# IGLICT/NeRFFaceEditing

Hardware: NVIDIA B200
Metric: rendered rays/sec (48+48 samples) (higher is better)
Workload: dtype f32 (gather, compositing) + bf16x3 split tensor-core MLP with f32 accumulate

## Files before the change

include/nfe_b200.h:

```cpp
#ifndef NFE_B200_H
#define NFE_B200_H

#include <stdint.h>

#ifdef __cplusplus
extern "C" {
#endif

typedef void* nfe_stream_t;

int nfe_version(void);
const char* nfe_last_error(void);
uint64_t nfe_launch_count(void);
int nfe_timing_enable(int on);
int nfe_timing_read(double* ms_by_stage, int64_t* count_by_stage, int n_stages, int reset);

int nfe_bench_l2_gather(const float* table, int64_t n_lines, int warps_per_cta, int depth, int iters, int64_t* host_lines_out,
                        float* sink, nfe_stream_t stream);

int nfe_plane_stats(const float* planes, int64_t n_slabs, int64_t hw, float* mean, float* std_out,
                    nfe_stream_t stream);
int nfe_plane_normalize(const float* planes, const float* mean, const float* std_in, int64_t n_slabs,
                        int64_t hw, float* out, nfe_stream_t stream);
int nfe_plane_denormalize(const float* norm, const float* mean, const float* std_in, int64_t n_slabs,
                          int64_t stat_slabs, int64_t hw, float* out, nfe_stream_t stream);
int nfe_plane_normalize_bwd(const float* g_norm, const float* norm, const float* std_in, const float* g_mean,
                            const float* g_std, int64_t n_slabs, int64_t hw, double* sums_ws, float* g_planes,
                            nfe_stream_t stream);
int nfe_resize_bilinear(const float* in, int64_t n_img, int in_h, int in_w, int out_h, int out_w, int antialias,
                        float* out, nfe_stream_t stream);
int nfe_planes_to_channel_last(const float* planes, int64_t n_img, int channels, int64_t hw, float* out,
                               nfe_stream_t stream);

int nfe_plane_normalize_staged(const float* planes, const float* mean, const float* std_in, int64_t n_img,
                               int64_t hw, float* out_norm, float* out_norm_cl, float* out_raw_cl,
                               nfe_stream_t stream);

int nfe_generate_rays(const float* cam2world , const float* intrinsics , int n,
                      int resolution, float* origins , float* dirs, nfe_stream_t stream);
int nfe_ray_limits_box(const float* origins, const float* dirs, int64_t n_rays, float box_side_length,
                       float* tmin, float* tmax, nfe_stream_t stream);

int nfe_sample_stratified(int64_t n_rays, int s_c, int mode, const float* table, double ray_start,
                          double ray_end, const float* start_per_ray, const float* end_per_ray,
                          const float* jitter, int stochastic, uint64_t seed, uint64_t offset,
                          float* depths , nfe_stream_t stream);

int nfe_sample_planes_fwd(const float* planes_cl, int plane_batch, int channels, int height, int width,
                          const float* coords , int n, int64_t m, float box_warp, float* out,
                          nfe_stream_t stream);

// ... 144 lines not shown
```

nerffaceediting_b200/_lib.py:

```python
import ctypes
import os

_HERE = os.path.dirname(os.path.abspath(__file__))
LIB_PATH = os.path.join(_HERE, "lib", "libnfe_b200.so")

DEC_OSG, DEC_DISENTANGLED, DEC_SEGMENTATION = 0, 1, 2
PREC_FP32, PREC_BF16X3, PREC_BF16 = 0, 1, 2

c_f32p = ctypes.c_void_p
c_i64 = ctypes.c_int64
c_u64 = ctypes.c_uint64
c_int = ctypes.c_int
c_float = ctypes.c_float
c_double = ctypes.c_double
c_vp = ctypes.c_void_p


class NfeMlp(ctypes.Structure):
    _fields_ = [("w1", c_vp), ("b1", c_vp), ("w2", c_vp), ("b2", c_vp),
                ("in_dim", c_int), ("hidden", c_int), ("out_dim", c_int),
                ("wgain1", c_float), ("bgain1", c_float), ("wgain2", c_float), ("bgain2", c_float)]


class NfeRenderCfg(ctypes.Structure):
# ... 13 lines not shown

_MLP_P = ctypes.POINTER(NfeMlp)
_CFG_P = ctypes.POINTER(NfeRenderCfg)

SIGNATURES = {
    "nfe_version": (c_int, []),
    "nfe_last_error": (ctypes.c_char_p, []),
    "nfe_launch_count": (c_u64, []),
    "nfe_timing_enable": (c_int, [c_int]),
    "nfe_timing_read": (c_int, [ctypes.POINTER(c_double), ctypes.POINTER(c_i64), c_int, c_int]),
    "nfe_bench_l2_gather": (c_int, [c_vp, c_i64, c_int, c_int, c_int, ctypes.POINTER(c_i64), c_vp, c_vp]),
    "nfe_plane_stats": (c_int, [c_vp, c_i64, c_i64, c_vp, c_vp, c_vp]),
    "nfe_plane_normalize": (c_int, [c_vp, c_vp, c_vp, c_i64, c_i64, c_vp, c_vp]),
    "nfe_plane_denormalize": (c_int, [c_vp, c_vp, c_vp, c_i64, c_i64, c_i64, c_vp, c_vp]),
    "nfe_plane_normalize_staged": (c_int, [c_vp, c_vp, c_vp, c_i64, c_i64, c_vp, c_vp, c_vp, c_vp]),
    "nfe_planes_to_channel_last": (c_int, [c_vp, c_i64, c_int, c_i64, c_vp, c_vp]),
    "nfe_generate_rays": (c_int, [c_vp, c_vp, c_int, c_int, c_vp, c_vp, c_vp]),
    "nfe_ray_limits_box": (c_int, [c_vp, c_vp, c_i64, c_float, c_vp, c_vp, c_vp]),
    "nfe_sample_stratified": (c_int, [c_i64, c_int, c_int, c_vp, c_double, c_double, c_vp, c_vp, c_vp, c_int, c_u64, c_u64, c_vp, c_vp]),
    "nfe_sample_planes_fwd": (c_int, [c_vp, c_int, c_int, c_int, c_int, c_vp, c_int, c_i64, c_float, c_vp, c_vp]),
    "nfe_decoder_fwd": (c_int, [c_int, c_int, _MLP_P, _MLP_P, c_vp, c_vp, c_int, c_i64, c_int, c_vp, c_vp, c_vp, c_vp]),
    "nfe_composite_fwd": (c_int, [c_vp, c_vp, c_vp, c_vp, c_i64, c_int, c_int, c_int, c_int, c_vp, c_vp, c_vp, c_vp, c_vp, c_vp, c_vp]),
    "nfe_importance_resample": (c_int, [c_vp, c_vp, c_i64, c_int, c_int, c_vp, c_int, c_u64, c_u64, c_vp, c_vp, c_vp, c_vp]),
    "nfe_sample_pdf": (c_int, [c_vp, c_vp, c_i64, c_int, c_int, c_int, c_vp, c_int, c_u64, c_u64, c_float, c_vp, c_vp]),
    "nfe_unify_samples":(c_int, [c_vp] * 8 + [c_i64, c_int, c_int, c_int, c_int] + [c_vp] * 4 + [c_vp]),
    "nfe_render_workspace_bytes": (c_i64, [_CFG_P, c_int, c_i64]),
    "nfe_render_fwd": (c_int, [_CFG_P, _MLP_P, _MLP_P, c_vp, c_vp, c_int, c_vp, c_vp, c_int, c_i64, c_vp, c_vp,
                               c_vp, c_vp, c_vp, c_vp, c_vp, c_int, c_vp, c_vp, c_vp, c_i64, c_vp]),
    "nfe_render_workspace_layout": (c_int, [_CFG_P, c_int, c_i64, ctypes.POINTER(c_i64)]),
    "nfe_composite_bwd": (c_int, [c_vp, c_vp, c_vp, c_int, c_vp, c_vp, c_vp, c_int, c_i64, c_int, c_int, c_vp, c_vp, c_vp, c_vp, c_vp, c_vp, c_vp, c_vp]),
# ... 66 lines not shown
```

nerffaceediting_b200/autograd.py:

```python
import ctypes
import os

import torch
import torch.nn.functional as F

from . import _lib, ops

MAX_ROWS = 1 << 22


def _mlp(x, seq):
    a, b = seq[0], seq[2]
    h = F.softplus(torch.addmm((a.bias * a.bias_gain).unsqueeze(0), x, (a.weight * a.weight_gain).t()))
    return torch.addmm((b.bias * b.bias_gain).unsqueeze(0), h, (b.weight * b.weight_gain).t())


def _decode(kind, seq_a, seq_b, fn, fd):
    if kind == ops.DEC_DISENTANGLED:
        g = _mlp(fn, seq_a)
        return g[:, :1], g[:, 1:], torch.sigmoid(_mlp(fd, seq_b)) * (1 + 2 * 0.001) - 0.001
    x = _mlp(fd, seq_a)
    rgb = torch.sigmoid(x[:, 1:]) * (1 + 2 * 0.001) - 0.001
    return x[:, :1], (_mlp(fd, seq_b) if kind == ops.DEC_SEGMENTATION else None), rgb

# ... 210 lines not shown
        if g.get("rgb") is not None:
            g_rec[:, 16:48] = g["rgb"].reshape(n * m, 32)
        with torch.cuda.device(dev):
            fb = _FieldBackward(kind, seq_a, seq_b, norm_cl, denorm_cl, ctx.affine, ctx.box_warp, ctx.needs_input_grad[5:], dev)
            fb.run_pass(n, rec, g_rec, coords=coords)
            norm_shape, plane_shape = ctx.plane_shapes
            g_norm, g_planes, g_scale, g_shift, g_params = fb.finish(norm_shape, plane_shape, ctx.needs_input_grad[1], ctx.needs_input_grad[2],
                                                                     ctx.stat_shapes, ctx.needs_input_grad[3], ctx.needs_input_grad[4])
        return (None, g_norm, g_planes, g_scale, g_shift) + tuple(g_params)


class NormalizeFunction(torch.autograd.Function):

    @staticmethod
    def forward(ctx, planes):
        mean, std = ops.plane_stats(planes)
        norm_cl = None
        if planes.dim() == 4 and planes.shape[1] == 96 and planes.is_contiguous() and planes.dtype == torch.float32:
            norm, norm_cl, _ = ops.plane_normalize_staged(planes.detach(), mean, std, register=False)
        else:
            norm = ops.plane_normalize(planes, mean, std)
        ctx.save_for_backward(norm, std)
        ctx.hw = planes.shape[-1] * planes.shape[-2]
        if norm_cl is None:
            return norm, mean, std, None
        ctx.mark_non_differentiable(norm_cl)
        return norm, mean, std, norm_cl

    @staticmethod
    def backward(ctx, g_norm, g_mean, g_std, _g_cl=None):
        norm, std = ctx.saved_tensors
        def f32(t):
            return None if t is None else t.contiguous().float()
        g, gm, gs = f32(g_norm), f32(g_mean), f32(g_std)
        slabs = norm.numel() // ctx.hw
        gx = torch.empty_like(norm)
        sums = torch.empty((slabs, 2), device=norm.device, dtype=torch.float64) if g is not None else None
        with torch.cuda.device(norm.device):
            _lib.check(_lib.load().nfe_plane_normalize_bwd(ops._ptr(g), ops._ptr(norm), ops._ptr(std), ops._ptr(gm), ops._ptr(gs), slabs, ctx.hw,
                                                           ops._ptr(sums), ops._ptr(gx), torch.cuda.current_stream(norm.device).cuda_stream),
                       "nfe_plane_normalize_bwd")
        return gx


class DenormalizeFunction(torch.autograd.Function):
# ... 20 lines not shown
```

nerffaceediting_b200/csrc/nfe_march.cu:

```cuda
#include "nfe_march.cuh"

namespace nfe {

__device__ __forceinline__ double shfl_up_double(double v, int delta)
{
    int lo = __double2loint(v), hi = __double2hiint(v);
    lo = __shfl_up_sync(0xffffffffu, lo, delta);
    hi = __shfl_up_sync(0xffffffffu, hi, delta);
    return __hiloint2double(hi, lo);
}
__device__ __forceinline__ double shfl_xor_double(double v, int mask)
{
    int lo = __double2loint(v), hi = __double2hiint(v);
    lo = __shfl_xor_sync(0xffffffffu, lo, mask);
    hi = __shfl_xor_sync(0xffffffffu, hi, mask);
    return __hiloint2double(hi, lo);
}

__device__ __forceinline__ void ray_interval_weights(const float* s_depth, const float* s_sigma, float* s_w, int S, int lane, float& wd, float& wt)
{
    const int n_int = S - 1;
    const int chunk = (n_int + 31) / 32;
    const int i0 = lane * chunk, i1 = min(n_int, i0 + chunk);
    float prod = 1.0f;
    for (int i = i0; i < i1; ++i) {
        const float delta = __fsub_rn(s_depth[i + 1], s_depth[i]);
        const float sig = __fdiv_rn(__fadd_rn(s_sigma[i], s_sigma[i + 1]), 2.0f);
        const float xs = __fsub_rn(sig, 1.0f);
        const float dens = fmaxf(xs, 0.0f) + __logf(1.0f + __expf(-fabsf(xs)));
        const float alpha = __fsub_rn(1.0f, __expf(-__fmul_rn(dens, delta)));
        s_w[i] = alpha;
        prod *= __fadd_rn(__fsub_rn(1.0f, alpha), 1e-10f);
    }
    float incl = prod;
#pragma unroll
    for (int o = 1; o < 32; o <<= 1) {
        const float up = __shfl_up_sync(0xffffffffu, incl, o);
        if (lane >= o) incl *= up;
    }
    float T = __shfl_up_sync(0xffffffffu, incl, 1);
    if (lane == 0) T = 1.0f;
    for (int i = i0; i < i1; ++i) {
        const float alpha = s_w[i];
        const float w = __fmul_rn(alpha, T);
        T *= __fadd_rn(__fsub_rn(1.0f, alpha), 1e-10f);
        s_w[i] = w;
        wd = fmaf(w, __fdiv_rn(__fadd_rn(s_depth[i], s_depth[i + 1]), 2.0f), wd);
        wt = __fadd_rn(wt, w);
    }
}

__device__ __forceinline__ void cp_async16(uint32_t dst_smem, const void* src)
{
    asm volatile("cp.async.cg.shared.global [%0], [%1], 16;" ::"r"(dst_smem), "l"(src) : "memory");
}
__device__ __forceinline__ void cp_async_commit() { asm volatile("cp.async.commit_group;" ::: "memory"); }
template <int N>
__device__ __forceinline__ void cp_async_wait() { asm volatile("cp.async.wait_group %0;" ::"n"(N) : "memory"); }

constexpr int MARCH_RING_GROUPS = 4;
constexpr int MARCH_MIN_BLOCKS = 4;
template <bool SORT>
__global__ void __launch_bounds__(256, MARCH_MIN_BLOCKS) march_kernel(MarchArgs a)
// ... 252 lines not shown
            const bool first = e < a.s1;
            const int64_t row = first ? ray * a.s1 + e : ray * a.s2 + (e - a.s1);
            for (int c = lane; c < a.cc; c += 32) colors_out[(ray * S + k) * a.cc + c] = (first ? a.colors1 : a.colors2)[row * a.cc + c];
            for (int c = lane; c < a.cs; c += 32) segs_out[(ray * S + k) * a.cs + c] = (first ? a.segs1 : a.segs2)[row * a.cs + c];
        }
        __syncwarp();
    }
}

constexpr int RESAMPLE_MIN_BLOCKS = 4;
template <bool SMOOTH>
__global__ void __launch_bounds__(256, RESAMPLE_MIN_BLOCKS) resample_kernel(ResampleArgs a)
{
    extern __shared__ __align__(16) float smem[];
    const int warp = threadIdx.x >> 5, lane = threadIdx.x & 31;
    const int warps_per_block = blockDim.x >> 5;
    const int S = a.S, nw = S - 1, ns = SMOOTH ? S - 3 : a.ns;
    const int per_warp = 4 * S + (a.sort_u ? a.s_f : 0);
    float* s_z = smem + (size_t)warp * per_warp;
    float* s_om = s_z + S;
    float* s_bins = s_om + S;
    float* s_cdf = s_bins + S;
    float* s_u = s_cdf + S;
    for (int64_t ray = (int64_t)blockIdx.x * warps_per_block + warp; ray < a.n_rays; ray += (int64_t)gridDim.x * warps_per_block) {
        if (SMOOTH) {
            for (int e = lane; e < S; e += 32) s_z[e] = a.z_vals[ray * S + e];
            if (a.sigma) {
                for (int e = lane; e < S; e += 32) s_om[e] = a.sigma[ray * S + e];
                __syncwarp();
                float wd = 0.0f, wt = 0.0f;
                ray_interval_weights(s_z, s_om, s_cdf, S, lane, wd, wt);
                __syncwarp();
                if (a.weights_out) for (int e = lane; e < nw; e += 32) a.weights_out[ray * nw + e] = s_cdf[e];
            } else {
                for (int e = lane; e < nw; e += 32) s_cdf[e] = a.weights[ray * nw + e];
            }
            __syncwarp();
            for (int i = lane; i < nw; i += 32) {
                const float w0 = s_cdf[i];
                const float m_i = i > 0 ? fmaxf(s_cdf[i - 1], w0) : w0;
                const float m_n = i + 1 < nw ? fmaxf(w0, s_cdf[i + 1]) : w0;
                const float sm = __fadd_rn(__fdiv_rn(__fadd_rn(m_i, m_n), 2.0f), 0.01f);
                if (i >= 1 && i <= ns) s_om[i - 1] = __fadd_rn(sm, a.eps);
                s_bins[i] = __fmul_rn(0.5f, __fadd_rn(s_z[i], s_z[i + 1]));
            }
        } else {
            for (int e = lane; e < S; e += 32) s_bins[e] = a.z_vals[ray * S + e];
            for (int e = lane; e < ns; e += 32) s_om[e] = __fadd_rn(a.weights[ray * ns + e], a.eps);
        }
        __syncwarp();
        double tot = 0.0;
        for (int j = lane; j < ns; j += 32) tot += (double)s_om[j];
#pragma unroll
        for (int o = 16; o > 0; o >>= 1) tot += shfl_xor_double(tot, o);
        const float totf = (float)tot;
        const int chunk = (ns + 31) / 32;
        const int j0 = lane * chunk, j1 = min(ns, j0 + chunk);
        double local = 0.0;
        for (int j = j0; j < j1; ++j) local += (double)__fdiv_rn(s_om[j], totf);
        double incl = local;
#pragma unroll
        for (int o = 1; o < 32; o <<= 1) {
            const double up = shfl_up_double(incl, o);
            if (lane >= o) incl += up;
        }
        double run = incl - local;
        __syncwarp();
        if (lane == 0) s_cdf[0] = 0.0f;
        for (int j = j0; j < j1; ++j) {
            run += (double)__fdiv_rn(s_om[j], totf);
            s_cdf[j + 1] = (float)run;
        }
        __syncwarp();
        const bool sort_u = a.sort_u && !a.u;
        if (sort_u) {
            for (int k = lane; k < a.s_f; k += 32) s_u[k] = u01(philox4x32(a.seed, (uint64_t)(ray * a.s_f + k), a.offset).x);
            __syncwarp();
        }
        for (int k = lane; k < a.s_f; k += 32) {
            float u;
            int dst = k;
            if (a.u) u = a.u_per_ray ? a.u[ray * a.s_f + k] : a.u[k];
            else if (sort_u) {
                u = s_u[k];
                dst = 0;
                for (int j = 0; j < a.s_f; ++j) {
                    const float uj = s_u[j];
                    dst += (uj < u) || (uj == u && j < k);
                }
            } else u = u01(philox4x32(a.seed, (uint64_t)(ray * a.s_f + k), a.offset).x);
            int lo = 0, hi = ns + 1;
            while (lo < hi) {
                const int mid = (lo + hi) >> 1;
                if (s_cdf[mid] <= u) lo = mid + 1; else hi = mid;
            }
            const int below = max(lo - 1, 0), above = min(lo, ns);
            float den = __fsub_rn(s_cdf[above], s_cdf[below]);
            if (den < a.eps) den = 1.0f;
            const float frac = __fdiv_rn(__fsub_rn(u, s_cdf[below]), den);
            const float t = __fadd_rn(s_bins[below], __fmul_rn(frac, __fsub_rn(s_bins[above], s_bins[below])));
            a.out[ray * a.s_f + dst] = t;
            if (a.below) a.below[ray * a.s_f + dst] = below;
            if (a.above) a.above[ray * a.s_f + dst] = above;
        }
        __syncwarp();
    }
}

static int warps_for(int S, int floats_per_sample)
{
    int w = 8;
    while (w > 1 && (size_t)w * floats_per_sample * 4 * S > 96 * 1024) w >>= 1;
    return w;
}

static constexpr size_t SMEM_OPT_IN = 40 * 1024;

int launch_march(const MarchArgs& a, bool sort, cudaStream_t stream)
// ... 25 lines not shown
}

int launch_finish_depth(float* depth, int64_t n, const float* minmax, cudaStream_t stream)
{
    if (n <= 0) return 0;
    finish_depth_kernel<<<(unsigned)((n + 255) / 256), 256, 0, stream>>>(depth, n, minmax);
    return check_launch("finish_depth_kernel");
}

int launch_resample(const ResampleArgs& a, cudaStream_t stream)
{
    NFE_REQUIRE(a.S >= (a.smooth ? 4 : 2) && a.S <= MAX_S, "importance resampling: %d bins unsupported (%d..%d)", a.S, a.smooth ? 4 : 2, MAX_S);
    NFE_REQUIRE(a.smooth || (a.ns >= 1 && a.ns < a.S), "sample_pdf: %d weights need at least %d bins (got %d)", a.ns, a.ns + 1, a.S);
    NFE_REQUIRE(a.s_f >= 1, "importance resampling: need at least one importance sample");
    if (a.n_rays <= 0) return 0;
    const int per_warp = 4 * a.S + (a.sort_u ? a.s_f : 0);
    int warps = 8;
    while (warps > 1 && (size_t)warps * per_warp * 4 > 96 * 1024) warps >>= 1;
    const size_t smem = (size_t)warps * per_warp * 4;
    const int64_t blocks = (a.n_rays + warps - 1) / warps;
    const int64_t cap = (int64_t)sm_count() * 8;
    const unsigned grid = (unsigned)(blocks < cap ? blocks : cap);
    if (a.smooth) {
        if (smem > SMEM_OPT_IN) cudaFuncSetAttribute(resample_kernel<true>, cudaFuncAttributeMaxDynamicSharedMemorySize, (int)smem);
        resample_kernel<true><<<grid, warps * 32, smem, stream>>>(a);
    } else {
        if (smem > SMEM_OPT_IN) cudaFuncSetAttribute(resample_kernel<false>, cudaFuncAttributeMaxDynamicSharedMemorySize, (int)smem);
        resample_kernel<false><<<grid, warps * 32, smem, stream>>>(a);
    }
    return check_launch("resample_kernel");
}

}

using namespace nfe;
// ... 77 lines not shown
```

nerffaceediting_b200/csrc/nfe_planes.cu:

```cuda
#include "nfe_common.cuh"

namespace nfe {

__global__ void __launch_bounds__(512) plane_stats_kernel(const float* __restrict__ planes, int64_t hw,
                                                          float* __restrict__ mean, float* __restrict__ std_out)
{
    const float* x = planes + (int64_t)blockIdx.x * hw;
    double s = 0.0, ss = 0.0;
    const bool vec = (hw % 4 == 0) && ((reinterpret_cast<uintptr_t>(x) & 15) == 0);
    if (vec) {
        const float4* x4 = reinterpret_cast<const float4*>(x);
        const int64_t n4 = hw / 4;
        for (int64_t i = threadIdx.x; i < n4; i += blockDim.x) {
            const float4 v = __ldg(x4 + i);
            s += (double)v.x; s += (double)v.y; s += (double)v.z; s += (double)v.w;
            ss += (double)v.x * (double)v.x; ss += (double)v.y * (double)v.y;
            ss += (double)v.z * (double)v.z; ss += (double)v.w * (double)v.w;
        }
    } else {
        for (int64_t i = threadIdx.x; i < hw; i += blockDim.x) {
            const double v = (double)x[i];
            s += v; ss += v * v;
        }
    }
#pragma unroll
    for (int o = 16; o > 0; o >>= 1) {
        s += __shfl_xor_sync(0xffffffffu, s, o);
        ss += __shfl_xor_sync(0xffffffffu, ss, o);
// ... 4 lines not shown
    __syncthreads();
    if (warp == 0) {
        const int nw = blockDim.x >> 5;
        s = lane < nw ? sh_s[lane] : 0.0;
        ss = lane < nw ? sh_ss[lane] : 0.0;
#pragma unroll
        for (int o = 8; o > 0; o >>= 1) {
            s += __shfl_xor_sync(0xffffffffu, s, o);
            ss += __shfl_xor_sync(0xffffffffu, ss, o);
        }
        if (lane == 0) {
            const double n = (double)hw;
            const double m = s / n;
            double var = (ss - s * m) / (n - 1.0);
            if (var < 0.0) var = 0.0;
            mean[blockIdx.x] = (float)m;
            std_out[blockIdx.x] = sqrtf((float)var);
        }
    }
}

__global__ void __launch_bounds__(256) plane_normalize_kernel(const float* __restrict__ planes, const float* __restrict__ mean,
                                                              const float* __restrict__ std_in, int64_t hw, int chunks_per_slab,
                                                              float* __restrict__ out)
{
    const int64_t slab = blockIdx.x / chunks_per_slab;
    const int chunk = blockIdx.x % chunks_per_slab;
    const float m = mean[slab];
    const float d = __fadd_rn(std_in[slab], 1e-8f);
    const int64_t per = (hw + chunks_per_slab - 1) / chunks_per_slab;
    const int64_t lo = chunk * per, hi = min(hw, lo + per);
    const float* x = planes + slab * hw;
    float* y = out + slab * hw;
    const bool vec = (hw % 4 == 0) && (per % 4 == 0) && (((reinterpret_cast<uintptr_t>(x) | reinterpret_cast<uintptr_t>(y)) & 15) == 0);
// ... 47 lines not shown
    const int64_t px0 = (blockIdx.x % tiles_per_img) * CL_PIX;
    const float* src = planes + img * channels * hw;
    float* dst = out + img * hw * channels;
    const int npx = (int)min((int64_t)CL_PIX, hw - px0);
    for (int i = threadIdx.x; i < channels * CL_PIX; i += blockDim.x) {
        const int c = i / CL_PIX, p = i % CL_PIX;
        if (p < npx) tile[c * (CL_PIX + 1) + p] = __ldg(src + (int64_t)c * hw + px0 + p);
    }
    __syncthreads();
    for (int i = threadIdx.x; i < npx * channels; i += blockDim.x) {
        const int p = i / channels, c = i % channels;
        dst[(px0 + p) * channels + c] = tile[c * (CL_PIX + 1) + p];
    }
}

constexpr int STAGE_MIN_BLOCKS = 4;
template <bool NORMALIZE>
__global__ void __launch_bounds__(256, STAGE_MIN_BLOCKS) stage32_kernel(const float* __restrict__ planes, const float* __restrict__ mean,
                                                      const float* __restrict__ std_in, int64_t hw, int64_t groups_per_img, int64_t n_groups,
                                                      float* __restrict__ out_norm, float* __restrict__ out_norm_cl, float* __restrict__ out_raw_cl)
{
    const int lane = threadIdx.x & 31;
    int64_t group = ((int64_t)blockIdx.x * blockDim.x + threadIdx.x) >> 5;
    if (group >= n_groups) return;
    if constexpr (NORMALIZE) group = n_groups - 1 - group;
    const int64_t img = group / groups_per_img;
    const int64_t px = (group % groups_per_img) * 32 + lane;
    const bool live = px < hw;
    const float* src = planes + img * 32 * hw + px;
    float x[32];
#pragma unroll
    for (int c = 0; c < 32; ++c) x[c] = live ? __ldg(src + (int64_t)c * hw) : 0.0f;
    if (live && out_raw_cl) {
        float4* dst = reinterpret_cast<float4*>(out_raw_cl + (img * hw + px) * 32);
#pragma unroll
        for (int q = 0; q < 8; ++q) dst[q] = make_float4(x[4 * q], x[4 * q + 1], x[4 * q + 2], x[4 * q + 3]);
    }
    if constexpr (NORMALIZE) {
        const float m_l = mean[img * 32 + lane];
        const float d_l = __fadd_rn(std_in[img * 32 + lane], 1e-8f);
#pragma unroll
        for (int c = 0; c < 32; ++c) {
            const float m = __shfl_sync(0xffffffffu, m_l, c), d = __shfl_sync(0xffffffffu, d_l, c);
            x[c] = __fdiv_rn(__fsub_rn(x[c], m), d);
        }
        if (live) {
            float* dn = out_norm + img * 32 * hw + px;
#pragma unroll
            for (int c = 0; c < 32; ++c) __stcs(dn + (int64_t)c * hw, x[c]);
            float4* dst = reinterpret_cast<float4*>(out_norm_cl + (img * hw + px) * 32);
#pragma unroll
            for (int q = 0; q < 8; ++q) dst[q] = make_float4(x[4 * q], x[4 * q + 1], x[4 * q + 2], x[4 * q + 3]);
        }
    }
}


__global__ void __launch_bounds__(512) plane_normalize_bwd_sums_kernel(const float* __restrict__ g, const float* __restrict__ norm, int64_t hw,
                                                                       double* __restrict__ sums)
{
    const float* gp = g + (int64_t)blockIdx.x * hw;
    const float* np_ = norm + (int64_t)blockIdx.x * hw;
    double s = 0.0, sn = 0.0;
    const bool vec = (hw % 4 == 0) && (((reinterpret_cast<uintptr_t>(gp) | reinterpret_cast<uintptr_t>(np_)) & 15) == 0);
    if (vec) {
        const float4* g4 = reinterpret_cast<const float4*>(gp);
        const float4* n4 = reinterpret_cast<const float4*>(np_);
// ... 120 lines not shown
{
    int64_t c = (int64_t)sm_count() * 16 / (n_slabs > 0 ? n_slabs : 1);
    const int64_t max_c = hw / 4096 > 0 ? hw / 4096 : 1;
    if (c > max_c) c = max_c;
    if (c < 1) c = 1;
    while (c > 1 && ((hw % c) != 0 || ((hw / c) % 4) != 0)) --c;
    return (int)c;
}

NFE_EXPORT int nfe_plane_stats(const float* planes, int64_t n_slabs, int64_t hw, float* mean, float* std_out, nfe_stream_t stream)
{
    if (n_slabs == 0) return 0;
    NFE_REQUIRE(planes && mean && std_out, "nfe_plane_stats: null pointer");
    NFE_REQUIRE(n_slabs >= 0 && n_slabs < (1ll << 31) && hw >= 2, "nfe_plane_stats: bad sizes (n_slabs=%lld hw=%lld)", (long long)n_slabs, (long long)hw);
    if (n_slabs == 0) return 0;
    plane_stats_kernel<<<(unsigned)n_slabs, 512, 0, as_stream(stream)>>>(planes, hw, mean, std_out);
    NFE_LAUNCH_CHECK("plane_stats_kernel");
    return 0;
}

NFE_EXPORT int nfe_plane_normalize(const float* planes, const float* mean, const float* std_in, int64_t n_slabs, int64_t hw,
                                   float* out, nfe_stream_t stream)
{
    if (n_slabs == 0 || hw == 0) return 0;
    NFE_REQUIRE(planes && mean && std_in && out, "nfe_plane_normalize: null pointer");
    NFE_REQUIRE(n_slabs >= 0 && hw >= 1, "nfe_plane_normalize: bad sizes");
    if (n_slabs == 0) return 0;
    const int chunks = chunks_for(n_slabs, hw);
    NFE_REQUIRE(n_slabs * chunks < (1ll << 31), "nfe_plane_normalize: grid too large");
    plane_normalize_kernel<<<(unsigned)(n_slabs * chunks), 256, 0, as_stream(stream)>>>(planes, mean, std_in, hw, chunks, out);
    NFE_LAUNCH_CHECK("plane_normalize_kernel");
// ... 40 lines not shown
NFE_EXPORT int nfe_plane_normalize_staged(const float* planes, const float* mean, const float* std_in, int64_t n_img, int64_t hw, float* out_norm,
                                          float* out_norm_cl, float* out_raw_cl, nfe_stream_t stream)
{
    if (n_img == 0 || hw == 0) return 0;
    NFE_REQUIRE(planes && mean && std_in && out_norm && out_norm_cl, "nfe_plane_normalize_staged: null pointer");
    NFE_REQUIRE(((reinterpret_cast<uintptr_t>(out_norm_cl) | reinterpret_cast<uintptr_t>(out_raw_cl)) & 15) == 0,
                "nfe_plane_normalize_staged: channel-last outputs must be 16-byte aligned");
    const int64_t groups_per_img = (hw + 31) / 32, n_groups = n_img * groups_per_img;
    NFE_REQUIRE((n_groups + 7) / 8 < (1ll << 31), "nfe_plane_normalize_staged: grid too large");
    stage32_kernel<true><<<(unsigned)((n_groups + 7) / 8), 256, 0, as_stream(stream)>>>(planes, mean, std_in, hw, groups_per_img, n_groups, out_norm,
                                                                                      out_norm_cl, out_raw_cl);
    NFE_LAUNCH_CHECK("stage32_kernel");
    return 0;
}

NFE_EXPORT int nfe_plane_normalize_bwd(const float* g_norm, const float* norm, const float* std_in, const float* g_mean, const float* g_std,
                                       int64_t n_slabs, int64_t hw, double* sums_ws, float* g_planes, nfe_stream_t stream)
{
    if (n_slabs == 0 || hw == 0) return 0;
    NFE_REQUIRE(norm && std_in && g_planes, "nfe_plane_normalize_bwd: null pointer");
    NFE_REQUIRE(!g_norm || sums_ws, "nfe_plane_normalize_bwd: the reduction workspace ([n_slabs,2] doubles) is missing");
    NFE_REQUIRE(n_slabs >= 0 && hw >= 2, "nfe_plane_normalize_bwd: bad sizes");
    NFE_REQUIRE(n_slabs < (1ll << 31), "nfe_plane_normalize_bwd: grid too large");
    if (g_norm) {
        plane_normalize_bwd_sums_kernel<<<(unsigned)n_slabs, 512, 0, as_stream(stream)>>>(g_norm, norm, hw, sums_ws);
        NFE_LAUNCH_CHECK("plane_normalize_bwd_sums_kernel");
    }
    const int chunks = chunks_for(n_slabs, hw);
    NFE_REQUIRE(n_slabs * chunks < (1ll << 31), "nfe_plane_normalize_bwd: grid too large");
    plane_normalize_bwd_apply_kernel<<<(unsigned)(n_slabs * chunks), 256, 0, as_stream(stream)>>>(g_norm, norm, std_in, g_mean, g_std, sums_ws, hw,
// ... 18 lines not shown
```

nerffaceediting_b200/ops.py:

```python
import ctypes

import os

import torch

from . import _lib
from . import plane_registry as registry
from ._lib import DEC_DISENTANGLED, DEC_OSG, DEC_SEGMENTATION, NfeMlp, NfeRenderCfg


def _cuda_f32(t, name):
    if not isinstance(t, torch.Tensor):
        raise RuntimeError(f"{name}: expected a tensor, got {type(t).__name__}")
    if not t.is_cuda:
        raise RuntimeError(f"{name}: expected a CUDA tensor (this path has no CPU fallback), got device {t.device}")
    if t.dtype != torch.float32:
        t = t.float()
    return t.contiguous()


def _ptr(t):
    return None if t is None else t.data_ptr()


# ... 117 lines not shown

def plane_normalize_staged(planes, mean, std, stage_raw=False, register=True):
    x = _cuda_f32(planes, "planes")
    n, c96, h, w = x.shape
    norm = torch.empty_like(x)
    norm_cl = torch.empty((n, 3, h, w, 32), device=x.device, dtype=torch.float32)
    raw_cl = torch.empty_like(norm_cl) if stage_raw else None
    with _Guard(x):
        _lib.check(_lib.load().nfe_plane_normalize_staged(_ptr(x), _ptr(mean), _ptr(std), n * 3, h * w, _ptr(norm), _ptr(norm_cl), _ptr(raw_cl),
                                                          _stream(x)), "nfe_plane_normalize_staged")
    if register:
        register_normalized(planes, norm, mean, std, norm_cl, raw_cl)
    return norm, norm_cl, raw_cl


def register_normalized(planes, norm, mean, std, norm_cl, raw_cl=None):
    n = planes.shape[0]
    registry.staged_put(norm, norm_cl)
    if raw_cl is not None:
        registry.staged_put(planes, raw_cl)
    registry.provenance_put(planes, norm, std.detach().reshape(n, -1) + 1e-8, mean.detach().reshape(n, -1))


def clear_plane_cache():
    registry.clear()


def generate_rays(cam2world, intrinsics, resolution):
    c = _cuda_f32(cam2world, "cam2world_matrix").reshape(-1, 16)
    k = _cuda_f32(intrinsics, "intrinsics").reshape(-1, 9)
    if c.shape[0] != k.shape[0]:
        raise RuntimeError("generate_rays: cam2world and intrinsics batch sizes differ")
    n, res = c.shape[0], int(resolution)
    o = torch.empty((n, res * res, 3), device=c.device, dtype=torch.float32)
    d = torch.empty_like(o)
    with _Guard(c):
# ... 373 lines not shown
```

nerffaceediting_b200/triplane.py:

```python
import numpy as np
import torch

from . import ops


class FullyConnectedLayer(torch.nn.Module):

    def __init__(self, in_features, out_features, bias=True, activation='linear', lr_multiplier=1, bias_init=0):
        super().__init__()
        assert activation == 'linear' and bias, "only the linear, biased layer of the decoders is provided"
        self.in_features = in_features
        self.out_features = out_features
        self.activation = activation
        self.weight = torch.nn.Parameter(torch.randn([out_features, in_features]) / lr_multiplier)
        self.bias = torch.nn.Parameter(torch.full([out_features], np.float32(bias_init)))
        self.weight_gain = lr_multiplier / np.sqrt(in_features)
        self.bias_gain = lr_multiplier

    def extra_repr(self):
        return f'in_features={self.in_features:d}, out_features={self.out_features:d}, activation={self.activation:s}'


def _mlp(n_features, hidden, out, lr_mul):
    return torch.nn.Sequential(FullyConnectedLayer(n_features, hidden, lr_multiplier=lr_mul), torch.nn.Softplus(),
# ... 35 lines not shown

    def forward(self, sampled_norm_features, sampled_denorm_features, ray_directions):
        ops._no_grad_needed(sampled_norm_features, sampled_denorm_features, *self.parameters())
        return ops.decoder_fwd(ops.DEC_DISENTANGLED, self.geo_net, self.app_net, sampled_norm_features, sampled_denorm_features)


def compute_mean_var(planes):
    ops._no_grad_needed(planes)
    return ops.plane_stats(planes)


def normalize_plane(planes):
    tri = planes.dim() == 4 and planes.shape[1] == 96 and planes.is_contiguous() and planes.dtype == torch.float32
    if torch.is_grad_enabled() and planes.requires_grad:
        from .autograd import NormalizeFunction
        norm, mean, std, norm_cl = NormalizeFunction.apply(planes)
        if norm_cl is not None:
            ops.register_normalized(planes, norm, mean, std, norm_cl)
            ops.provenance_attach(planes, std, 1e-8, mean)
        return norm, mean, std
    mean, std = ops.plane_stats(planes)
    if tri:
        return ops.plane_normalize_staged(planes, mean, std)[0], mean, std
    return ops.plane_normalize(planes, mean, std), mean, std


def denormalize_plane(planes, mean, var):
    if torch.is_grad_enabled() and any(torch.is_tensor(t) and t.requires_grad for t in (planes, mean, var)):
        from .autograd import DenormalizeFunction
        out = DenormalizeFunction.apply(planes, mean, var)
        if torch.is_tensor(mean) and torch.is_tensor(var):
            ops.register_denormalized(out, planes, mean, var)
            ops.provenance_attach(out, var, 0.0, mean, norm_requires_grad=planes.requires_grad)
        return out
    return ops.plane_denormalize(planes, mean, var)


class TriPlaneGenerator(torch.nn.Module):
# ... 97 lines not shown
```

Baseline: 33.92 million.

## Fuse plane stats and normalization into one persistent kernel; half-warp PDF sampling

Replaces the separate plane-stats and staged-normalize launches with one persistent kernel. It hands out stats units and normalize units through an atomic ticket, and each normalize unit waits on a per-image counter until that image's 32 slab stats are done. This is meant to overlap the stats reduction with normalization and remove a launch and a serialization point. Separately, importance sampling now processes two rays per warp (16 lanes each), with float and native double shuffles replacing the emulated double shuffles. The stats loop also batches its float4 loads. The risks are spin-wait deadlock if the scheduling assumptions fail, and lower per-ray parallelism on long rays.

```diff
diff --git a/include/nfe_b200.h b/include/nfe_b200.h
--- a/include/nfe_b200.h
+++ b/include/nfe_b200.h
@@ -35,6 +35,9 @@
 int nfe_plane_normalize_staged(const float* planes, const float* mean, const float* std_in, int64_t n_img,
                                int64_t hw, float* out_norm, float* out_norm_cl, float* out_raw_cl,
                                nfe_stream_t stream);
+
+int nfe_plane_prepare(const float* planes, int64_t n_img, int64_t hw, float* mean, float* std_out, float* scale,
+                      float* out_norm, float* out_norm_cl, float* out_raw_cl, int32_t* counters_ws, nfe_stream_t stream);
 
 int nfe_generate_rays(const float* cam2world , const float* intrinsics , int n,
                       int resolution, float* origins , float* dirs, nfe_stream_t stream);
diff --git a/nerffaceediting_b200/_lib.py b/nerffaceediting_b200/_lib.py
--- a/nerffaceediting_b200/_lib.py
+++ b/nerffaceediting_b200/_lib.py
@@ -51,6 +51,7 @@
     "nfe_plane_normalize": (c_int, [c_vp, c_vp, c_vp, c_i64, c_i64, c_vp, c_vp]),
     "nfe_plane_denormalize": (c_int, [c_vp, c_vp, c_vp, c_i64, c_i64, c_i64, c_vp, c_vp]),
     "nfe_plane_normalize_staged": (c_int, [c_vp, c_vp, c_vp, c_i64, c_i64, c_vp, c_vp, c_vp, c_vp]),
+    "nfe_plane_prepare": (c_int, [c_vp, c_i64, c_i64, c_vp, c_vp, c_vp, c_vp, c_vp, c_vp, c_vp, c_vp]),
     "nfe_planes_to_channel_last": (c_int, [c_vp, c_i64, c_int, c_i64, c_vp, c_vp]),
     "nfe_generate_rays": (c_int, [c_vp, c_vp, c_int, c_int, c_vp, c_vp, c_vp]),
     "nfe_ray_limits_box": (c_int, [c_vp, c_vp, c_i64, c_float, c_vp, c_vp, c_vp]),
diff --git a/nerffaceediting_b200/autograd.py b/nerffaceediting_b200/autograd.py
--- a/nerffaceediting_b200/autograd.py
+++ b/nerffaceediting_b200/autograd.py
@@ -248,21 +248,21 @@
 
     @staticmethod
     def forward(ctx, planes):
-        mean, std = ops.plane_stats(planes)
-        norm_cl = None
         if planes.dim() == 4 and planes.shape[1] == 96 and planes.is_contiguous() and planes.dtype == torch.float32:
-            norm, norm_cl, _ = ops.plane_normalize_staged(planes.detach(), mean, std, register=False)
+            norm, mean, std, scale, norm_cl, _ = ops.plane_prepare(planes.detach(), register=False)
         else:
+            mean, std = ops.plane_stats(planes)
             norm = ops.plane_normalize(planes, mean, std)
+            norm_cl = scale = None
         ctx.save_for_backward(norm, std)
         ctx.hw = planes.shape[-1] * planes.shape[-2]
         if norm_cl is None:
-            return norm, mean, std, None
-        ctx.mark_non_differentiable(norm_cl)
-        return norm, mean, std, norm_cl
-
-    @staticmethod
-    def backward(ctx, g_norm, g_mean, g_std, _g_cl=None):
+            return norm, mean, std, None, None
+        ctx.mark_non_differentiable(norm_cl, scale)
+        return norm, mean, std, norm_cl, scale
+
+    @staticmethod
+    def backward(ctx, g_norm, g_mean, g_std, _g_cl=None, _g_scale=None):
         norm, std = ctx.saved_tensors
         def f32(t):
             return None if t is None else t.contiguous().float()
diff --git a/nerffaceediting_b200/csrc/nfe_march.cu b/nerffaceediting_b200/csrc/nfe_march.cu
--- a/nerffaceediting_b200/csrc/nfe_march.cu
+++ b/nerffaceediting_b200/csrc/nfe_march.cu
@@ -2,19 +2,13 @@
 
 namespace nfe {
 
-__device__ __forceinline__ double shfl_up_double(double v, int delta)
-{
-    int lo = __double2loint(v), hi = __double2hiint(v);
-    lo = __shfl_up_sync(0xffffffffu, lo, delta);
-    hi = __shfl_up_sync(0xffffffffu, hi, delta);
-    return __hiloint2double(hi, lo);
-}
-__device__ __forceinline__ double shfl_xor_double(double v, int mask)
-{
-    int lo = __double2loint(v), hi = __double2hiint(v);
-    lo = __shfl_xor_sync(0xffffffffu, lo, mask);
-    hi = __shfl_xor_sync(0xffffffffu, hi, mask);
-    return __hiloint2double(hi, lo);
+__device__ __forceinline__ float interval_alpha(const float* s_depth, const float* s_sigma, int i)
+{
+    const float delta = __fsub_rn(s_depth[i + 1], s_depth[i]);
+    const float sig = __fdiv_rn(__fadd_rn(s_sigma[i], s_sigma[i + 1]), 2.0f);
+    const float xs = __fsub_rn(sig, 1.0f);
+    const float dens = fmaxf(xs, 0.0f) + __logf(1.0f + __expf(-fabsf(xs)));
+    return __fsub_rn(1.0f, __expf(-__fmul_rn(dens, delta)));
 }
 
 __device__ __forceinline__ void ray_interval_weights(const float* s_depth, const float* s_sigma, float* s_w, int S, int lane, float& wd, float& wt)
@@ -24,11 +18,7 @@
     const int i0 = lane * chunk, i1 = min(n_int, i0 + chunk);
     float prod = 1.0f;
     for (int i = i0; i < i1; ++i) {
-        const float delta = __fsub_rn(s_depth[i + 1], s_depth[i]);
-        const float sig = __fdiv_rn(__fadd_rn(s_sigma[i], s_sigma[i + 1]), 2.0f);
-        const float xs = __fsub_rn(sig, 1.0f);
-        const float dens = fmaxf(xs, 0.0f) + __logf(1.0f + __expf(-fabsf(xs)));
-        const float alpha = __fsub_rn(1.0f, __expf(-__fmul_rn(dens, delta)));
+        const float alpha = interval_alpha(s_depth, s_sigma, i);
         s_w[i] = alpha;
         prod *= __fadd_rn(__fsub_rn(1.0f, alpha), 1e-10f);
     }
@@ -47,6 +37,45 @@
         s_w[i] = w;
         wd = fmaf(w, __fdiv_rn(__fadd_rn(s_depth[i], s_depth[i + 1]), 2.0f), wd);
         wt = __fadd_rn(wt, w);
+    }
+}
+
+__device__ __forceinline__ void ray_interval_weights_half(const float* s_depth, const float* s_sigma, float* s_w, int S, int q)
+{
+    const int n_int = S - 1;
+    const int chunk = (n_int + 31) / 32;
+    float p[2];
+#pragma unroll
+    for (int v = 0; v < 2; ++v) {
+        const int i0 = (2 * q + v) * chunk, i1 = min(n_int, i0 + chunk);
+        float prod = 1.0f;
+        for (int i = i0; i < i1; ++i) {
+            const float alpha = interval_alpha(s_depth, s_sigma, i);
+            s_w[i] = alpha;
+            prod *= __fadd_rn(__fsub_rn(1.0f, alpha), 1e-10f);
+        }
+        p[v] = prod;
+    }
+    {
+        const float up = __shfl_up_sync(0xffffffffu, p[1], 1, 16);
+        p[1] *= p[0];
+        if (q >= 1) p[0] *= up;
+    }
+#pragma unroll
+    for (int o = 2; o < 32; o <<= 1) {
+        const float u0 = __shfl_up_sync(0xffffffffu, p[0], o / 2, 16), u1 = __shfl_up_sync(0xffffffffu, p[1], o / 2, 16);
+        if (2 * q >= o) { p[0] *= u0; p[1] *= u1; }
+    }
+    const float up = __shfl_up_sync(0xffffffffu, p[1], 1, 16);
+#pragma unroll
+    for (int v = 0; v < 2; ++v) {
+        float T = v ? p[0] : (q >= 1 ? up : 1.0f);
+        const int i0 = (2 * q + v) * chunk, i1 = min(n_int, i0 + chunk);
+        for (int i = i0; i < i1; ++i) {
+            const float alpha = s_w[i];
+            s_w[i] = __fmul_rn(alpha, T);
+            T *= __fadd_rn(__fsub_rn(1.0f, alpha), 1e-10f);
+        }
     }
 }
 
@@ -329,29 +358,32 @@
 {
     extern __shared__ __align__(16) float smem[];
     const int warp = threadIdx.x >> 5, lane = threadIdx.x & 31;
+    const int half = lane >> 4, q = lane & 15;
     const int warps_per_block = blockDim.x >> 5;
     const int S = a.S, nw = S - 1, ns = SMOOTH ? S - 3 : a.ns;
-    const int per_warp = 4 * S + (a.sort_u ? a.s_f : 0);
-    float* s_z = smem + (size_t)warp * per_warp;
+    const int per_ray = 4 * S + (a.sort_u ? a.s_f : 0);
+    float* s_z = smem + (size_t)(2 * warp + half) * per_ray;
     float* s_om = s_z + S;
     float* s_bins = s_om + S;
     float* s_cdf = s_bins + S;
     float* s_u = s_cdf + S;
-    for (int64_t ray = (int64_t)blockIdx.x * warps_per_block + warp; ray < a.n_rays; ray += (int64_t)gridDim.x * warps_per_block) {
+    const int64_t stride = 2 * (int64_t)gridDim.x * warps_per_block;
+    for (int64_t ray0 = 2 * ((int64_t)blockIdx.x * warps_per_block + warp); ray0 < a.n_rays; ray0 += stride) {
+        const bool live = ray0 + half < a.n_rays;
+        const int64_t ray = live ? ray0 + half : ray0;
         if (SMOOTH) {
-            for (int e = lane; e < S; e += 32) s_z[e] = a.z_vals[ray * S + e];
+            for (int e = q; e < S; e += 16) s_z[e] = a.z_vals[ray * S + e];
             if (a.sigma) {
-                for (int e = lane; e < S; e += 32) s_om[e] = a.sigma[ray * S + e];
+                for (int e = q; e < S; e += 16) s_om[e] = a.sigma[ray * S + e];
                 __syncwarp();
-                float wd = 0.0f, wt = 0.0f;
-                ray_interval_weights(s_z, s_om, s_cdf, S, lane, wd, wt);
+                ray_interval_weights_half(s_z, s_om, s_cdf, S, q);
                 __syncwarp();
-                if (a.weights_out) for (int e = lane; e < nw; e += 32) a.weights_out[ray * nw + e] = s_cdf[e];
+                if (a.weights_out && live) for (int e = q; e < nw; e += 16) a.weights_out[ray * nw + e] = s_cdf[e];
             } else {
-                for (int e = lane; e < nw; e += 32) s_cdf[e] = a.weights[ray * nw + e];
+                for (int e = q; e < nw; e += 16) s_cdf[e] = a.weights[ray * nw + e];
             }
             __syncwarp();
-            for (int i = lane; i < nw; i += 32) {
+            for (int i = q; i < nw; i += 16) {
                 const float w0 = s_cdf[i];
                 const float m_i = i > 0 ? fmaxf(s_cdf[i - 1], w0) : w0;
                 const float m_n = i + 1 < nw ? fmaxf(w0, s_cdf[i + 1]) : w0;
@@ -360,28 +392,27 @@
                 s_bins[i] = __fmul_rn(0.5f, __fadd_rn(s_z[i], s_z[i + 1]));
             }
         } else {
-            for (int e = lane; e < S; e += 32) s_bins[e] = a.z_vals[ray * S + e];
-            for (int e = lane; e < ns; e += 32) s_om[e] = __fadd_rn(a.weights[ray * ns + e], a.eps);
-        }
-        __syncwarp();
+            for (int e = q; e < S; e += 16) s_bins[e] = a.z_vals[ray * S + e];
+            for (int e = q; e < ns; e += 16) s_om[e] = __fadd_rn(a.weights[ray * ns + e], a.eps);
+        }
+        __syncwarp();
+        const int chunk = (ns + 15) / 16;
+        const int j0 = q * chunk, j1 = min(ns, j0 + chunk);
         double tot = 0.0;
-        for (int j = lane; j < ns; j += 32) tot += (double)s_om[j];
-#pragma unroll
-        for (int o = 16; o > 0; o >>= 1) tot += shfl_xor_double(tot, o);
+        for (int j = j0; j < j1; ++j) tot += (double)s_om[j];
+#pragma unroll
+        for (int o = 8; o > 0; o >>= 1) tot += __shfl_xor_sync(0xffffffffu, tot, o, 16);
         const float totf = (float)tot;
-        const int chunk = (ns + 31) / 32;
-        const int j0 = lane * chunk, j1 = min(ns, j0 + chunk);
         double local = 0.0;
         for (int j = j0; j < j1; ++j) local += (double)__fdiv_rn(s_om[j], totf);
         double incl = local;
 #pragma unroll
-        for (int o = 1; o < 32; o <<= 1) {
-            const double up = shfl_up_double(incl, o);
-            if (lane >= o) incl += up;
+        for (int o = 1; o < 16; o <<= 1) {
+            const double up = __shfl_up_sync(0xffffffffu, incl, o, 16);
+            if (q >= o) incl += up;
         }
         double run = incl - local;
-        __syncwarp();
-        if (lane == 0) s_cdf[0] = 0.0f;
+        if (q == 0) s_cdf[0] = 0.0f;
         for (int j = j0; j < j1; ++j) {
             run += (double)__fdiv_rn(s_om[j], totf);
             s_cdf[j + 1] = (float)run;
@@ -389,10 +420,10 @@
         __syncwarp();
         const bool sort_u = a.sort_u && !a.u;
         if (sort_u) {
-            for (int k = lane; k < a.s_f; k += 32) s_u[k] = u01(philox4x32(a.seed, (uint64_t)(ray * a.s_f + k), a.offset).x);
+            for (int k = q; k < a.s_f; k += 16) s_u[k] = u01(philox4x32(a.seed, (uint64_t)(ray * a.s_f + k), a.offset).x);
             __syncwarp();
         }
-        for (int k = lane; k < a.s_f; k += 32) {
+        for (int k = q; k < a.s_f; k += 16) {
             float u;
             int dst = k;
             if (a.u) u = a.u_per_ray ? a.u[ray * a.s_f + k] : a.u[k];
@@ -414,9 +445,11 @@
             if (den < a.eps) den = 1.0f;
             const float frac = __fdiv_rn(__fsub_rn(u, s_cdf[below]), den);
             const float t = __fadd_rn(s_bins[below], __fmul_rn(frac, __fsub_rn(s_bins[above], s_bins[below])));
-            a.out[ray * a.s_f + dst] = t;
-            if (a.below) a.below[ray * a.s_f + dst] = below;
-            if (a.above) a.above[ray * a.s_f + dst] = above;
+            if (live) {
+                a.out[ray * a.s_f + dst] = t;
+                if (a.below) a.below[ray * a.s_f + dst] = below;
+                if (a.above) a.above[ray * a.s_f + dst] = above;
+            }
         }
         __syncwarp();
     }
@@ -472,11 +505,11 @@
     NFE_REQUIRE(a.smooth || (a.ns >= 1 && a.ns < a.S), "sample_pdf: %d weights need at least %d bins (got %d)", a.ns, a.ns + 1, a.S);
     NFE_REQUIRE(a.s_f >= 1, "importance resampling: need at least one importance sample");
     if (a.n_rays <= 0) return 0;
-    const int per_warp = 4 * a.S + (a.sort_u ? a.s_f : 0);
+    const int per_ray = 4 * a.S + (a.sort_u ? a.s_f : 0);
     int warps = 8;
-    while (warps > 1 && (size_t)warps * per_warp * 4 > 96 * 1024) warps >>= 1;
-    const size_t smem = (size_t)warps * per_warp * 4;
-    const int64_t blocks = (a.n_rays + warps - 1) / warps;
+    while (warps > 1 && (size_t)warps * 2 * per_ray * 4 > 96 * 1024) warps >>= 1;
+    const size_t smem = (size_t)warps * 2 * per_ray * 4;
+    const int64_t blocks = (a.n_rays + 2 * warps - 1) / (2 * warps);
     const int64_t cap = (int64_t)sm_count() * 8;
     const unsigned grid = (unsigned)(blocks < cap ? blocks : cap);
     if (a.smooth) {
diff --git a/nerffaceediting_b200/csrc/nfe_planes.cu b/nerffaceediting_b200/csrc/nfe_planes.cu
--- a/nerffaceediting_b200/csrc/nfe_planes.cu
+++ b/nerffaceediting_b200/csrc/nfe_planes.cu
@@ -1,17 +1,31 @@
+#include <cuda/atomic>
+
 #include "nfe_common.cuh"
 
 namespace nfe {
 
-__global__ void __launch_bounds__(512) plane_stats_kernel(const float* __restrict__ planes, int64_t hw,
-                                                          float* __restrict__ mean, float* __restrict__ std_out)
-{
-    const float* x = planes + (int64_t)blockIdx.x * hw;
+constexpr int STATS_THREADS = 512;
+__device__ __forceinline__ void block_slab_stats(const float* __restrict__ x, int64_t hw, float* mean, float* std_out, float* scale)
+{
     double s = 0.0, ss = 0.0;
     const bool vec = (hw % 4 == 0) && ((reinterpret_cast<uintptr_t>(x) & 15) == 0);
     if (vec) {
         const float4* x4 = reinterpret_cast<const float4*>(x);
         const int64_t n4 = hw / 4;
-        for (int64_t i = threadIdx.x; i < n4; i += blockDim.x) {
+        int64_t i = threadIdx.x;
+        constexpr int BATCH = 8;
+        for (; i + (BATCH - 1) * (int64_t)blockDim.x < n4; i += BATCH * (int64_t)blockDim.x) {
+            float4 v[BATCH];
+#pragma unroll
+            for (int b = 0; b < BATCH; ++b) v[b] = __ldg(x4 + i + b * (int64_t)blockDim.x);
+#pragma unroll
+            for (int b = 0; b < BATCH; ++b) {
+                s += (double)v[b].x; s += (double)v[b].y; s += (double)v[b].z; s += (double)v[b].w;
+                ss += (double)v[b].x * (double)v[b].x; ss += (double)v[b].y * (double)v[b].y;
+                ss += (double)v[b].z * (double)v[b].z; ss += (double)v[b].w * (double)v[b].w;
+            }
+        }
+        for (; i < n4; i += blockDim.x) {
             const float4 v = __ldg(x4 + i);
             s += (double)v.x; s += (double)v.y; s += (double)v.z; s += (double)v.w;
             ss += (double)v.x * (double)v.x; ss += (double)v.y * (double)v.y;
@@ -46,10 +60,19 @@
             const double m = s / n;
             double var = (ss - s * m) / (n - 1.0);
             if (var < 0.0) var = 0.0;
-            mean[blockIdx.x] = (float)m;
-            std_out[blockIdx.x] = sqrtf((float)var);
-        }
-    }
+            const float sd = sqrtf((float)var);
+            *mean = (float)m;
+            *std_out = sd;
+            if (scale) *scale = __fadd_rn(sd, 1e-8f);
+        }
+    }
+    __syncthreads();
+}
+
+__global__ void __launch_bounds__(STATS_THREADS) plane_stats_kernel(const float* __restrict__ planes, int64_t hw, float* __restrict__ mean,
+                                                                    float* __restrict__ std_out, float* __restrict__ scale)
+{
+    block_slab_stats(planes + (int64_t)blockIdx.x * hw, hw, mean + blockIdx.x, std_out + blockIdx.x, scale ? scale + blockIdx.x : nullptr);
 }
 
 __global__ void __launch_bounds__(256) plane_normalize_kernel(const float* __restrict__ planes, const float* __restrict__ mean,
@@ -127,6 +150,37 @@
     }
 }
 
+template <bool NORMALIZE>
+__device__ __forceinline__ void stage32_warp(const float* __restrict__ planes, int64_t img, int64_t px, int64_t hw, float m_l, float d_l,
+                                             float* __restrict__ out_norm, float* __restrict__ out_norm_cl, float* __restrict__ out_raw_cl)
+{
+    const bool live = px < hw;
+    const float* src = planes + img * 32 * hw + px;
+    float x[32];
+#pragma unroll
+    for (int c = 0; c < 32; ++c) x[c] = live ? __ldg(src + (int64_t)c * hw) : 0.0f;
+    if (live && out_raw_cl) {
+        float4* dst = reinterpret_cast<float4*>(out_raw_cl + (img * hw + px) * 32);
+#pragma unroll
+        for (int q = 0; q < 8; ++q) dst[q] = make_float4(x[4 * q], x[4 * q + 1], x[4 * q + 2], x[4 * q + 3]);
+    }
+    if constexpr (NORMALIZE) {
+#pragma unroll
+        for (int c = 0; c < 32; ++c) {
+            const float m = __shfl_sync(0xffffffffu, m_l, c), d = __shfl_sync(0xffffffffu, d_l, c);
+            x[c] = __fdiv_rn(__fsub_rn(x[c], m), d);
+        }
+        if (live) {
+            float* dn = out_norm + img * 32 * hw + px;
+#pragma unroll
+            for (int c = 0; c < 32; ++c) __stcs(dn + (int64_t)c * hw, x[c]);
+            float4* dst = reinterpret_cast<float4*>(out_norm_cl + (img * hw + px) * 32);
+#pragma unroll
+            for (int q = 0; q < 8; ++q) dst[q] = make_float4(x[4 * q], x[4 * q + 1], x[4 * q + 2], x[4 * q + 3]);
+        }
+    }
+}
+
 constexpr int STAGE_MIN_BLOCKS = 4;
 template <bool NORMALIZE>
 __global__ void __launch_bounds__(256, STAGE_MIN_BLOCKS) stage32_kernel(const float* __restrict__ planes, const float* __restrict__ mean,
@@ -139,31 +193,68 @@
     if constexpr (NORMALIZE) group = n_groups - 1 - group;
     const int64_t img = group / groups_per_img;
     const int64_t px = (group % groups_per_img) * 32 + lane;
-    const bool live = px < hw;
-    const float* src = planes + img * 32 * hw + px;
-    float x[32];
-#pragma unroll
-    for (int c = 0; c < 32; ++c) x[c] = live ? __ldg(src + (int64_t)c * hw) : 0.0f;
-    if (live && out_raw_cl) {
-        float4* dst = reinterpret_cast<float4*>(out_raw_cl + (img * hw + px) * 32);
-#pragma unroll
-        for (int q = 0; q < 8; ++q) dst[q] = make_float4(x[4 * q], x[4 * q + 1], x[4 * q + 2], x[4 * q + 3]);
-    }
+    float m_l = 0.0f, d_l = 0.0f;
     if constexpr (NORMALIZE) {
-        const float m_l = mean[img * 32 + lane];
-        const float d_l = __fadd_rn(std_in[img * 32 + lane], 1e-8f);
-#pragma unroll
-        for (int c = 0; c < 32; ++c) {
-            const float m = __shfl_sync(0xffffffffu, m_l, c), d = __shfl_sync(0xffffffffu, d_l, c);
-            x[c] = __fdiv_rn(__fsub_rn(x[c], m), d);
-        }
-        if (live) {
-            float* dn = out_norm + img * 32 * hw + px;
-#pragma unroll
-            for (int c = 0; c < 32; ++c) __stcs(dn + (int64_t)c * hw, x[c]);
-            float4* dst = reinterpret_cast<float4*>(out_norm_cl + (img * hw + px) * 32);
-#pragma unroll
-            for (int q = 0; q < 8; ++q) dst[q] = make_float4(x[4 * q], x[4 * q + 1], x[4 * q + 2], x[4 * q + 3]);
+        m_l = mean[img * 32 + lane];
+        d_l = __fadd_rn(std_in[img * 32 + lane], 1e-8f);
+    }
+    stage32_warp<NORMALIZE>(planes, img, px, hw, m_l, d_l, out_norm, out_norm_cl, out_raw_cl);
+}
+
+constexpr int PREP_THREADS = STATS_THREADS;
+constexpr int PREP_PIX = (PREP_THREADS / 32) * 32;
+constexpr int PREP_MIN_BLOCKS = 2;
+
+struct PrepArgs {
+    const float* planes; int64_t hw; int64_t n_img, units_per_img, lag;
+    float* mean; float* std_out; float* scale;
+    float* out_norm; float* out_norm_cl; float* out_raw_cl;
+    int* counters;
+};
+
+__global__ void __launch_bounds__(PREP_THREADS, PREP_MIN_BLOCKS) plane_prepare_kernel(PrepArgs a)
+{
+    __shared__ int s_ticket;
+    const int64_t G = a.n_img, U = a.units_per_img, L = a.lag;
+    const int64_t total = G * (32 + U);
+    const int warp = threadIdx.x >> 5, lane = threadIdx.x & 31;
+    for (;;) {
+        if (threadIdx.x == 0) s_ticket = atomicAdd(a.counters, 1);
+        __syncthreads();
+        const int64_t t = s_ticket;
+        if (t >= total) return;
+        bool stats;
+        int64_t walk, unit;
+        const int64_t mid = (G - L) * (32 + U);
+        if (t < 32 * L) {
+            stats = true; walk = t / 32; unit = t % 32;
+        } else if (t - 32 * L < mid) {
+            const int64_t w = L + (t - 32 * L) / (32 + U), r = (t - 32 * L) % (32 + U);
+            stats = r < 32;
+            walk = stats ? w : w - L;
+            unit = stats ? r : r - 32;
+        } else {
+            const int64_t t3 = t - 32 * L - mid;
+            stats = false; walk = G - L + t3 / U; unit = t3 % U;
+        }
+        const int64_t g = G - 1 - walk;
+        cuda::atomic_ref<int, cuda::thread_scope_device> done(a.counters[1 + g]);
+        if (stats) {
+            const int64_t slab = g * 32 + unit;
+            block_slab_stats(a.planes + slab * a.hw, a.hw, a.mean + slab, a.std_out + slab, a.scale + slab);
+            if (threadIdx.x == 0) done.fetch_add(1, cuda::memory_order_release);
+        } else {
+            if (threadIdx.x == 0) {
+                while (done.load(cuda::memory_order_acquire) < 32) __nanosleep(100);
+            }
+            __syncthreads();
+            const int64_t px0 = unit * PREP_PIX + warp * 32;
+            if (px0 < a.hw) {
+                const float m_l = __ldcg(a.mean + g * 32 + lane);
+                const float d_l = __ldcg(a.scale + g * 32 + lane);
+                stage32_warp<true>(a.planes, g, px0 + lane, a.hw, m_l, d_l, a.out_norm, a.out_norm_cl, a.out_raw_cl);
+            }
+            __syncthreads();
         }
     }
 }
@@ -314,7 +405,7 @@
     NFE_REQUIRE(planes && mean && std_out, "nfe_plane_stats: null pointer");
     NFE_REQUIRE(n_slabs >= 0 && n_slabs < (1ll << 31) && hw >= 2, "nfe_plane_stats: bad sizes (n_slabs=%lld hw=%lld)", (long long)n_slabs, (long long)hw);
     if (n_slabs == 0) return 0;
-    plane_stats_kernel<<<(unsigned)n_slabs, 512, 0, as_stream(stream)>>>(planes, hw, mean, std_out);
+    plane_stats_kernel<<<(unsigned)n_slabs, STATS_THREADS, 0, as_stream(stream)>>>(planes, hw, mean, std_out, nullptr);
     NFE_LAUNCH_CHECK("plane_stats_kernel");
     return 0;
 }
@@ -385,6 +476,46 @@
     return 0;
 }
 
+static bool plane_prepare_fused(const float* planes, int64_t hw)
+{
+    return hw % 4 == 0 && (reinterpret_cast<uintptr_t>(planes) & 15) == 0;
+}
+
+NFE_EXPORT int nfe_plane_prepare(const float* planes, int64_t n_img, int64_t hw, float* mean, float* std_out, float* scale, float* out_norm,
+                                 float* out_norm_cl, float* out_raw_cl, int32_t* counters_ws, nfe_stream_t stream)
+{
+    if (n_img == 0) return 0;
+    NFE_REQUIRE(planes && mean && std_out && scale && out_norm && out_norm_cl && counters_ws, "nfe_plane_prepare: null pointer");
+    NFE_REQUIRE(n_img > 0 && n_img * 32 < (1ll << 31) && hw >= 2, "nfe_plane_prepare: bad sizes (n_img=%lld hw=%lld)", (long long)n_img, (long long)hw);
+    NFE_REQUIRE(((reinterpret_cast<uintptr_t>(out_norm_cl) | reinterpret_cast<uintptr_t>(out_raw_cl)) & 15) == 0,
+                "nfe_plane_prepare: channel-last outputs must be 16-byte aligned");
+    cudaStream_t st = as_stream(stream);
+    if (!plane_prepare_fused(planes, hw)) {
+        plane_stats_kernel<<<(unsigned)(n_img * 32), STATS_THREADS, 0, st>>>(planes, hw, mean, std_out, scale);
+        NFE_LAUNCH_CHECK("plane_stats_kernel");
+        return nfe_plane_normalize_staged(planes, mean, std_out, n_img, hw, out_norm, out_norm_cl, out_raw_cl, stream);
+    }
+    static int per_sm = 0;
+    if (!per_sm) {
+        if (cudaOccupancyMaxActiveBlocksPerMultiprocessor(&per_sm, plane_prepare_kernel, PREP_THREADS, 0) != cudaSuccess || per_sm < 1) per_sm = 1;
+    }
+    PrepArgs a;
+    a.planes = planes; a.hw = hw; a.n_img = n_img; a.units_per_img = (hw + PREP_PIX - 1) / PREP_PIX;
+    const int64_t resident = (int64_t)sm_count() * per_sm, total = n_img * (32 + a.units_per_img);
+    const int64_t lag = resident / (32 + a.units_per_img) + 2;
+    a.lag = lag < n_img ? lag : n_img;
+    a.mean = mean; a.std_out = std_out; a.scale = scale; a.out_norm = out_norm; a.out_norm_cl = out_norm_cl; a.out_raw_cl = out_raw_cl;
+    a.counters = counters_ws;
+    NFE_REQUIRE(total < (1ll << 31), "nfe_plane_prepare: too many work units");
+    if (cudaError_t e = cudaMemsetAsync(counters_ws, 0, (size_t)(n_img + 1) * sizeof(int32_t), st)) {
+        set_error("nfe_plane_prepare: counter reset: %s", cudaGetErrorString(e));
+        return 1;
+    }
+    plane_prepare_kernel<<<(unsigned)(total < resident ? total : resident), PREP_THREADS, 0, st>>>(a);
+    NFE_LAUNCH_CHECK("plane_prepare_kernel");
+    return 0;
+}
+
 NFE_EXPORT int nfe_plane_normalize_bwd(const float* g_norm, const float* norm, const float* std_in, const float* g_mean, const float* g_std,
                                        int64_t n_slabs, int64_t hw, double* sums_ws, float* g_planes, nfe_stream_t stream)
 {
diff --git a/nerffaceediting_b200/ops.py b/nerffaceediting_b200/ops.py
--- a/nerffaceediting_b200/ops.py
+++ b/nerffaceediting_b200/ops.py
@@ -155,12 +155,32 @@
     return norm, norm_cl, raw_cl
 
 
-def register_normalized(planes, norm, mean, std, norm_cl, raw_cl=None):
+def plane_prepare(planes, stage_raw=False, register=True):
+    x = _cuda_f32(planes, "planes")
+    n, c96, h, w = x.shape
+    mean = torch.empty((n, c96, 1, 1), device=x.device, dtype=torch.float32)
+    std = torch.empty_like(mean)
+    scale = torch.empty((n, c96), device=x.device, dtype=torch.float32)
+    norm = torch.empty_like(x)
+    norm_cl = torch.empty((n, 3, h, w, 32), device=x.device, dtype=torch.float32)
+    raw_cl = torch.empty_like(norm_cl) if stage_raw else None
+    counters = torch.empty(n * 3 + 1, device=x.device, dtype=torch.int32)
+    with _Guard(x):
+        _lib.check(_lib.load().nfe_plane_prepare(_ptr(x), n * 3, h * w, _ptr(mean), _ptr(std), _ptr(scale), _ptr(norm), _ptr(norm_cl),
+                                                 _ptr(raw_cl), _ptr(counters), _stream(x)), "nfe_plane_prepare")
+    if register:
+        register_normalized(planes, norm, mean, std, norm_cl, raw_cl, scale=scale)
+    return norm, mean, std, scale, norm_cl, raw_cl
+
+
+def register_normalized(planes, norm, mean, std, norm_cl, raw_cl=None, scale=None):
     n = planes.shape[0]
     registry.staged_put(norm, norm_cl)
     if raw_cl is not None:
         registry.staged_put(planes, raw_cl)
-    registry.provenance_put(planes, norm, std.detach().reshape(n, -1) + 1e-8, mean.detach().reshape(n, -1))
+    if scale is None:
+        scale = std.detach().reshape(n, -1) + 1e-8
+    registry.provenance_put(planes, norm, scale, mean.detach().reshape(n, -1))
 
 
 def clear_plane_cache():
diff --git a/nerffaceediting_b200/triplane.py b/nerffaceediting_b200/triplane.py
--- a/nerffaceediting_b200/triplane.py
+++ b/nerffaceediting_b200/triplane.py
@@ -73,14 +73,15 @@
     tri = planes.dim() == 4 and planes.shape[1] == 96 and planes.is_contiguous() and planes.dtype == torch.float32
     if torch.is_grad_enabled() and planes.requires_grad:
         from .autograd import NormalizeFunction
-        norm, mean, std, norm_cl = NormalizeFunction.apply(planes)
+        norm, mean, std, norm_cl, scale = NormalizeFunction.apply(planes)
         if norm_cl is not None:
-            ops.register_normalized(planes, norm, mean, std, norm_cl)
+            ops.register_normalized(planes, norm, mean, std, norm_cl, scale=scale)
             ops.provenance_attach(planes, std, 1e-8, mean)
         return norm, mean, std
+    if tri:
+        norm, mean, std = ops.plane_prepare(planes)[:3]
+        return norm, mean, std
     mean, std = ops.plane_stats(planes)
-    if tri:
-        return ops.plane_normalize_staged(planes, mean, std)[0], mean, std
     return ops.plane_normalize(planes, mean, std), mean, std
 
 
```

After: 34.23 million (median of 6 runs). No clear change (+0.9%).
